# keeffEoghan/tendrils

Hardware: AMD Instinct MI355X
Metric: particle-steps/sec (16M particles per GPU) (higher is better)
Workload: dtype f32

## Files before the change

include/tendrils_hip.h:

```cpp
#ifndef TENDRILS_HIP_H
#define TENDRILS_HIP_H

#include <stddef.h>
#include <stdint.h>

#ifdef __cplusplus
extern "C" {
#endif

#define TH_ABI_VERSION 14

typedef int32_t th_status;
enum {
    TH_OK = 0,
    TH_ERR_INVALID = 1,
    TH_ERR_HIP = 2,
    TH_ERR_NO_DEVICE = 3,
    TH_ERR_UNSUPPORTED = 4
};

#define TH_INERT (-1000000.0f)

typedef struct th_context th_context;

// ... 171 lines not shown
} th_render_uniforms;
th_status th_view_draw(th_context *ctx, const th_render_uniforms *u, uint64_t *fragments);
th_status th_draw(th_context *ctx, const th_deposit_uniforms *u, const th_render_uniforms *r, uint64_t *fragments);
th_status th_view_fill(th_context *ctx, const float rgba[4]);
th_status th_view_clear(th_context *ctx);
th_status th_view_download(th_context *ctx, uint8_t *rgba8);
th_status th_view_buffers(th_context *ctx, int32_t count);
th_status th_view_bind(th_context *ctx, int32_t index);
th_status th_view_copy(th_context *ctx, int32_t index);
th_status th_view_step_buffers(th_context *ctx);
th_status th_colormap_upload(th_context *ctx, const float *rgba, int32_t w, int32_t h);
th_status th_export_view_lines(th_context *ctx, const th_render_uniforms *u, float *lines, uint64_t capacity, uint64_t *count);
th_status th_draw_sharded(th_context *ctx, const th_deposit_uniforms *u, const th_render_uniforms *r, uint64_t *fragments);
th_status th_view_emit(th_context *ctx, const th_render_uniforms *u, uint64_t *count, void **keys_dev, void **colors_dev);
th_status th_view_merge(th_context *ctx, const void *keys_dev, const void *colors_dev, uint64_t count);
th_status th_view_device_ptr(th_context *ctx, void **dptr);
th_status th_draw_emit(th_context *ctx, const th_deposit_uniforms *u, const th_render_uniforms *r, uint64_t *count, void **keys_dev, void **colors_dev);
th_status th_draw_merge(th_context *ctx, const void *keys_dev, const void *colors_dev, uint64_t count);

typedef struct th_slot_order_info {
    int32_t sorted_buffers;
    int32_t steps_since_sort;
    uint64_t window_misses;
    uint64_t sorts;
} th_slot_order_info;
th_status th_slot_order(th_context *ctx, th_slot_order_info *out);

enum { TH_DRAW_AUTO = -1, TH_DRAW_STREAM = 0, TH_DRAW_BINS = 1 };
th_status th_draw_pipeline(th_context *ctx, int32_t which);
typedef struct th_draw_info {
    int32_t pipeline;
    int32_t reserved;
    uint64_t fragments, crowded_fragments;
    uint64_t sent_bytes, received_bytes;
} th_draw_info;
th_status th_draw_query(th_context *ctx, th_draw_info *out);

typedef struct th_flow_line_uniforms {
    float speed, rad, crestShape, speedLimit;
    float viewSize[2];
} th_flow_line_uniforms;

th_status th_flow_line_attributes(const float *points, const double *times, int32_t n, int32_t closed, int32_t capacity,
                                  int32_t *nverts, float *position, float *normal, float *miter, float *previous,
                                  float *time, float *dt);
th_status th_flow_lines(th_context *ctx, const th_flow_line_uniforms *u, const float *points, const double *times,
                        const int32_t *offsets, const int32_t *closed, int32_t nlines);

enum { TH_OPT_BUCKET = 0, TH_OPT_RESORT_STEPS = 1, TH_OPT_REBUCKET_STEPS = 2, TH_OPT_FUSE = 3, TH_OPT_GRAPH = 4,
       TH_OPT_FORCE_GENERIC = 5, TH_OPT_DRAW_REUSE = 6, TH_OPT_BINS_POOL = 7,
#ifdef TH_TESTING
       TH_OPT_INJECT_FAILURE = 8,
#endif
       TH_OPT_BINS_PAGES = 9, TH_OPT_ASYNC_SORT = 10, TH_OPT_SKIP_UNSEEN = 11, TH_OPT_SPAWN_CHUNK_ROWS = 12 };
th_status th_option_set(th_context *ctx, int32_t option, int64_t value);
th_status th_option_get(th_context *ctx, int32_t option, int64_t *value);

#ifdef __cplusplus
}
#endif
#endif
```

tendrils_amd/csrc/th_api.hip:

```cpp
#include "th_ctx.hpp"

using namespace thi;

namespace {

thread_local std::string g_error;

void build_gradient_table(float4 *lut)
{
    for (int a = th::kLutMin; a <= th::kLutMax; ++a) {
        float p = th::permute_ref((float)a);
        float gx, gy, gz;
        th::gradient_ref(p, gx, gy, gz);
        lut[a - th::kLutMin] = make_float4(gx, gy, gz, 0.0f);
    }
}

void options_from_environment(th_options &o)
{
    auto number = [](const char *name, long long otherwise) { const char *e = getenv(name); return e && *e ? atoll(e) : otherwise; };
    o.bucket = (int)number("TH_BUCKET", -1);
    o.resort_steps = (int)number("TH_RESORT_STEPS", 64); if (o.resort_steps <= 0) o.resort_steps = 64;
    o.rebucket_steps = (int)number("TH_REBUCKET_STEPS", 256); if (o.rebucket_steps <= 0) o.rebucket_steps = 256;
    o.fuse = number("TH_FUSE", 1) != 0;
    o.graph = number("TH_GRAPH", 1) != 0;
    o.force_generic = getenv("TH_FORCE_GENERIC") != nullptr && number("TH_FORCE_GENERIC", 1) != 0;
    const char *d = getenv("TH_DRAW");
    o.draw = !d ? -1 : (!strcmp(d, "bins") ? 1 : (!strcmp(d, "stream") ? 0 : -1));
    o.draw_reuse = number("TH_DRAW_REUSE", 1) != 0;
    o.async_sort = number("TH_ASYNC_SORT", 1) != 0;
    o.skip_unseen = number("TH_SKIP_UNSEEN", 1) != 0;
    o.spawn_chunk_rows = (int)number("TH_SPAWN_CHUNK_ROWS", 0); if (o.spawn_chunk_rows < 0) o.spawn_chunk_rows = 0;
    o.bins_pool = (uint32_t)number("TH_BINS_POOL", 0);
    o.bins_pages = (int)number("TH_BINS_PAGES", 0); if (o.bins_pages > (int)th::kBinPagesLimit || o.bins_pages < -(int)th::kBinPagesLimit) o.bins_pages = 0;
}

}

namespace thi {

std::string &last_error() { return g_error; }

th_status fail(th_status code, const char *fmt, ...)
{
    char buf[512];
    va_list ap;
    va_start(ap, fmt);
    vsnprintf(buf, sizeof buf, fmt, ap);
    va_end(ap);
    g_error = buf;
    return code;
}

th_status use(th_context *c, bool keeps_lines)
{
    if (!c) return fail(TH_ERR_INVALID, "null context");
    TH_HIP(hipSetDevice(c->cfg.device));
    if (!keeps_lines) { c->drawn.valid = false; c->fused_stats.valid = false; }
    return TH_OK;
}

th_status alloc_state(th_context *c, float4 **out)
{
    TH_HIP(hipMalloc((void **)out, c->state_bytes()));
    TH_HIP(hipMemsetAsync(*out, 0, c->state_bytes(), c->stream));
    return TH_OK;
}

th_status resolve_target(th_context *c, int32_t target, bool rotate_ok, float4 **out)
{
    if (target == TH_TARGET_RING) {
        if (!rotate_ok) return fail(TH_ERR_INVALID, "TH_TARGET_RING not valid here");
        float4 *last = c->ring.back();
        c->ring.pop_back();
        c->ring.insert(c->ring.begin(), last);
        *out = c->ring[0];
        state_written(c, *out);
// ... 462 lines not shown
th_status th_timer_stop(th_context *c, float *elapsed_ms)
{
    if (th_status s = use(c, true)) return s;
    TH_REQUIRE(elapsed_ms, "null output");
    TH_HIP(hipEventRecord(c->ev1, c->stream));
    TH_HIP(hipEventSynchronize(c->ev1));
    TH_HIP(hipEventElapsedTime(elapsed_ms, c->ev0, c->ev1));
    return TH_OK;
}

th_status th_kernel_timing(th_context *c, int32_t enable)
{
    if (th_status s = use(c, true)) return s;
    c->kernel_timing = enable != 0;
    if (!enable) c->kt_used = 0;
    return TH_OK;
}

th_status th_kernel_timing_read(th_context *c, float *mean_ms, int32_t *launches)
{
    if (th_status s = use(c, true)) return s;
    TH_REQUIRE(mean_ms && launches, "null output");
    TH_HIP(hipStreamSynchronize(c->stream));
    double sum = 0.0;
    for (size_t k = 0; k + 1 < c->kt_used; k += 2) {
        float ms = 0.0f;
        TH_HIP(hipEventElapsedTime(&ms, c->kt_events[k], c->kt_events[k + 1]));
        sum += ms;
    }
    *launches = (int32_t)(c->kt_used / 2);
    *mean_ms = *launches ? (float)(sum / *launches) : 0.0f;
    c->kt_used = 0;
    return TH_OK;
}

th_status th_shapes(th_context *c, th_shapes_info *out)
{
    TH_REQUIRE(c && out, "null argument");
    out->state_w = c->cfg.width; out->state_h = c->cfg.height;
    out->flow_w = c->fw; out->flow_h = c->fh;
    out->frames_w = c->frw; out->frames_h = c->frh;
    return TH_OK;
}

th_status th_option_set(th_context *c, int32_t option, int64_t value)
{
    if (th_status s = use(c)) return s;
    th_options &o = c->opt;
    switch (option) {
    case TH_OPT_BUCKET: TH_REQUIRE(value >= -1 && value <= 1, "TH_OPT_BUCKET takes -1, 0 or 1"); o.bucket = (int)value; break;
    case TH_OPT_RESORT_STEPS: TH_REQUIRE(value > 0 && value < (1 << 30), "TH_OPT_RESORT_STEPS must be positive"); o.resort_steps = (int)value; break;
    case TH_OPT_REBUCKET_STEPS: TH_REQUIRE(value > 0 && value < (1 << 30), "TH_OPT_REBUCKET_STEPS must be positive"); o.rebucket_steps = (int)value; break;
    case TH_OPT_FUSE: o.fuse = value != 0; break;
    case TH_OPT_GRAPH: o.graph = value != 0; break;
    case TH_OPT_FORCE_GENERIC: o.force_generic = value != 0; break;
    case TH_OPT_DRAW_REUSE: o.draw_reuse = value != 0; break;
    case TH_OPT_SKIP_UNSEEN: o.skip_unseen = value != 0; break;
    case TH_OPT_ASYNC_SORT: o.async_sort = value != 0; if (!o.async_sort) { if (th_status s = asort_drop(c)) return s; } break;
    case TH_OPT_BINS_POOL: TH_REQUIRE(value >= 0 && value < (1ll << 32), "TH_OPT_BINS_POOL out of range"); o.bins_pool = (uint32_t)value; break;
#ifdef TH_TESTING
    case TH_OPT_INJECT_FAILURE: TH_REQUIRE(value >= 0 && value <= 5, "TH_OPT_INJECT_FAILURE takes 0..5"); o.inject_failure = (int)value; break;
#endif
    case TH_OPT_SPAWN_CHUNK_ROWS: TH_REQUIRE(value >= 0 && value < (1 << 30), "TH_OPT_SPAWN_CHUNK_ROWS takes 0 (by the scratch budget) or a number of rows"); o.spawn_chunk_rows = (int)value; break;
    case TH_OPT_BINS_PAGES:
        TH_REQUIRE(value >= -(int64_t)th::kBinPagesLimit && value <= (int64_t)th::kBinPagesLimit && value != 1 && value != -1, "TH_OPT_BINS_PAGES takes 0, or 2..%u (negative: never widened)", th::kBinPagesLimit);
        o.bins_pages = (int)value;
        if (c->chunk_table) {
            TH_HIP(hipStreamSynchronize(c->stream));
            (void)hipFree(c->chunk_table); c->chunk_table = nullptr; (void)hipFree(c->bin_mem); c->bin_mem = nullptr; c->bin_capacity = 0; c->bin_max_pages = 0;
        }
        break;
    default: return fail(TH_ERR_INVALID, "unknown option %d", option);
    }
    clear_graphs(c);
    return TH_OK;
}

th_status th_option_get(th_context *c, int32_t option, int64_t *value)
{
    TH_REQUIRE(c && value, "null argument");
    const th_options &o = c->opt;
    switch (option) {
    case TH_OPT_BUCKET: *value = o.bucket; break;
    case TH_OPT_RESORT_STEPS: *value = o.resort_steps; break;
    case TH_OPT_REBUCKET_STEPS: *value = o.rebucket_steps; break;
    case TH_OPT_FUSE: *value = o.fuse; break;
    case TH_OPT_GRAPH: *value = o.graph; break;
    case TH_OPT_FORCE_GENERIC: *value = o.force_generic; break;
    case TH_OPT_DRAW_REUSE: *value = o.draw_reuse; break;
    case TH_OPT_ASYNC_SORT: *value = o.async_sort; break;
    case TH_OPT_SKIP_UNSEEN: *value = o.skip_unseen; break;
    case TH_OPT_BINS_POOL: *value = o.bins_pool; break;
#ifdef TH_TESTING
    case TH_OPT_INJECT_FAILURE: *value = o.inject_failure; break;
#endif
    case TH_OPT_BINS_PAGES: *value = o.bins_pages; break;
    case TH_OPT_SPAWN_CHUNK_ROWS: *value = o.spawn_chunk_rows; break;
    default: return fail(TH_ERR_INVALID, "unknown option %d", option);
    }
    return TH_OK;
}

}
```

tendrils_amd/csrc/th_ctx.hpp:

```cpp
#pragma once
#include <hip/hip_runtime.h>

#include <algorithm>
#include <cmath>
#include <cstdarg>
#include <cstdio>
#include <cstdlib>
#include <cstring>
#include <limits>
#include <new>
#include <string>
#include <vector>

#include "th_kernels.hpp"
#include "th_math.hpp"

namespace thi {
struct FlowLineScratch;
th_status fail(th_status code, const char *fmt, ...);
std::string &last_error();
}

#define TH_HIP(expr)                                                                            \
    do {                                                                                        \
        hipError_t e_ = (expr);                                                                 \
        if (e_ != hipSuccess)                                                                   \
            return thi::fail(TH_ERR_HIP, "%s failed: %s (%s:%d)", #expr, hipGetErrorString(e_), __FILE__, __LINE__); \
    } while (0)

#define TH_REQUIRE(cond, ...)                            \
    do {                                                 \
        if (!(cond)) return thi::fail(TH_ERR_INVALID, __VA_ARGS__); \
    } while (0)

struct th_options {
    int bucket = -1;
    int resort_steps = 64;
    int rebucket_steps = 256;
    bool fuse = true;
    bool graph = true;
    bool force_generic = false;
    int draw = -1;
    bool draw_reuse = true;
    uint32_t bins_pool = 0;
    int bins_pages = 0;
    int inject_failure = 0;
    bool skip_unseen = true;
    int spawn_chunk_rows = 0;
    bool async_sort = true;
};

struct GraphEntry {
    int32_t n = 0;
    th::LogicVariant variant{};
    bool generic = false;
    std::vector<float4 *> ring;
    th::LogicParams key{};
    hipGraphExec_t exec = nullptr;
    float *times_dev = nullptr, *times_host = nullptr;
    hipEvent_t copied = nullptr;
};

struct th_context {
    th_config cfg{};
    th_options opt{};
    hipStream_t stream = nullptr;
    std::vector<float4 *> ring;
    bool packed = false;
    float4 *tmp[3] = {nullptr, nullptr, nullptr};
    float4 *flow = nullptr;
    float2 *flow_dec = nullptr;
    float *flow3 = nullptr;
    int32_t fw = 0, fh = 0;
    float4 *targets = nullptr;
    bool targets_checked = true, targets_nonfinite = false;
    float4 *lut = nullptr, *lut_block = nullptr;
    uchar4 *frames[2] = {nullptr, nullptr};
    int32_t frw = 0, frh = 0;
    unsigned int *d_flag = nullptr;
    th::StatsPartial *partials = nullptr;
    th::StatsPartial *fused_parts = nullptr;
    uint32_t fused_parts_cap = 0;
    struct { bool valid = false; const float4 *buf = nullptr; float limit = 0.0f; uint32_t nparts = 0; } fused_stats;
    th_counters *d_counters = nullptr;
    float4 *x_halo = nullptr;
    unsigned long long *x_counts = nullptr;
    unsigned long long *x_keys = nullptr;
    float4 *x_colors = nullptr;
    size_t x_capacity = 0;
    float4 *gathered = nullptr;
    const void *gathered_of = nullptr;
    void *sp_taps = nullptr;
// ... 208 lines not shown
```

tendrils_amd/csrc/th_kernels.hip:

```cpp
#include "th_kernels.hpp"
#include "th_math.hpp"
#include "th_logic.hpp"

#include <type_traits>
#include <cstdlib>

namespace th {


static int grid_for(size_t n, int blocks_per_cu)
{
    size_t blocks = (n + 255) / 256;
    size_t cap = (size_t)256 * blocks_per_cu;
    return (int)(blocks < cap ? (blocks ? blocks : 1) : cap);
}



__global__ __launch_bounds__(256) void pack_state_kernel(uint2 *dst, const float4 *src, uint32_t n)
{
    for (uint32_t i = blockIdx.x * 256u + threadIdx.x; i < n; i += gridDim.x * 256u) dst[i] = pack_state(src[i]);
}

__global__ __launch_bounds__(256) void unpack_state_kernel(float4 *dst, const uint2 *src, uint32_t n)
// ... 102 lines not shown
    if (b) lift([&](auto... c) { f(std::true_type{}, c...); }, rest...);
    else lift([&](auto... c) { f(std::false_type{}, c...); }, rest...);
}

void launch_logic(const LogicParams &p, const LogicVariant &v, hipStream_t s)
{
    const bool packed = v.format == StateFormat::packed;
    const int grid = packed ? grid_for(p.count, p.perm ? 20 : 8) : grid_for(p.count, 20);
    lift([&](auto fast, auto noise, auto target, auto pow2, auto decoded, auto perm) {
        constexpr bool ptab = noise && perm;
        hipLaunchKernelGGL((packed ? logic_packed_kernel<fast, noise, target, pow2, decoded, ptab>
                                   : logic_kernel<fast, noise, target, pow2, decoded, ptab>), dim3(grid), dim3(256), 0, s, p);
    }, v.mode == TH_MODE_FAST, v.noise, v.target, v.pow2, v.decoded, p.perm != nullptr);
}

void launch_logic_generic(const LogicParams &p, hipStream_t s)
{
    hipLaunchKernelGGL(logic_generic_kernel, dim3(grid_for(p.count, 8)), dim3(256), 0, s, p);
}

TH_D void stats_take(StatsPartial *slot, const float4 &v, float limit, bool first)
{
    const float cap = limit * (1.0f - 9.5367431640625e-07f);
    const bool is_live = v.x != kInert || v.y != kInert;
    const bool is_nan = (v.x != v.x) || (v.y != v.y) || (v.z != v.z) || (v.w != v.w);
    const float sp = __builtin_sqrtf(v.z * v.z + v.w * v.w);
    const bool fin = is_live && !is_nan && sp <= 3.4028234e38f;
    StatsPartial t;
    t.live = __builtin_popcountll(__ballot(is_live)); t.nan = __builtin_popcountll(__ballot(is_nan));
    t.capped = __builtin_popcountll(__ballot(fin && sp >= cap));
    double sum = fin ? (double)sp : 0.0;
    float mx = fin ? sp : 0.0f;
#pragma unroll
    for (int o = 32; o > 0; o >>= 1) {
        sum += __shfl_xor(sum, o);
        const float om = __shfl_xor(mx, o); mx = om > mx ? om : mx;
    }
    if (__lane_id() == (uint32_t)__builtin_ctzll(__ballot(true))) {
        t.sum_speed = sum; t.max_speed = (double)mx;
        if (!first) {
            const StatsPartial o = *slot;
            t.live += o.live; t.nan += o.nan; t.capped += o.capped; t.sum_speed += o.sum_speed;
            t.max_speed = o.max_speed > t.max_speed ? o.max_speed : t.max_speed;
        }
        *slot = t;
    }
}

TH_D void stats_none(StatsPartial *slot, bool first)
{
    if (__ballot(!first) == 0ull && __lane_id() == 0u) *slot = StatsPartial{0ull, 0ull, 0ull, 0.0, 0.0};
}

#define TH_LOGIC_FUSED_LOOP(Fmt)                                                                                              \
    __shared__ float4 smem[NOISE ? kHashVec + kLutSize : 1];                                                                  \
    const float4 *lut = smem + (NOISE ? kHashVec : 0);                                                                        \
    const HashTables tabs{reinterpret_cast<const uint32_t *>(smem), reinterpret_cast<const uint32_t *>(smem) + kPermA};       \
    if constexpr (NOISE) {                                                                                                    \
        fill_hash_tables(smem, p.lut);                                                                                        \
        __syncthreads();                                                                                                      \
    }                                                                                                                         \
    uint32_t idx, stride, end;                                                                                                \
    if constexpr (!BUCKETED) {                                                                                                \
        idx = blockIdx.x * 256u + threadIdx.x;                                                                                \
        stride = gridDim.x * 256u;                                                                                            \
        end = p.count;                                                                                                        \
    } else {                                                                                                                  \
        const uint32_t group = blockIdx.x & 7u, rank = blockIdx.x >> 3, per = (p.count + 7u) >> 3;                            \
        const uint32_t lo = group * per;                                                                                      \
        idx = lo + rank * 256u + threadIdx.x;                                                                                 \
        stride = (gridDim.x >> 3) * 256u;                                                                                     \
        end = lo + per < p.count ? lo + per : p.count;                                                                        \
    }                                                                                                                         \
    typename Fmt::Word nxt = Fmt::empty();                                                                                    \
    uint32_t npid = idx;                                                                                                      \
    [[maybe_unused]] bool first = true;                                                                                       \
    if (idx < end) {                                                                                                          \
        nxt = Fmt::load(p.in, idx);                                                                                           \
        if constexpr (BUCKETED) npid = __builtin_nontemporal_load(&p.perm[idx]);                                              \
    }                                                                                                                         \
    for (; idx < end; idx += stride) {                                                                                        \
        typename Fmt::Word w = nxt, wprev = w;                                                                                \
        const uint32_t pid = BUCKETED ? npid : idx;                                                                           \
        if (idx + stride < end) {                                                                                             \
            nxt = Fmt::load(p.in, idx + stride);                                                                              \
            if constexpr (BUCKETED) npid = __builtin_nontemporal_load(&p.perm[idx + stride]);                                 \
        }                                                                                                                     \
        float4 st = Fmt::decode(w);                                                                                           \
        for (uint32_t k = 0; k < p.nsteps; ++k) {                                                                             \
            if constexpr (!Fmt::packed) wprev = Fmt::encode(st);                                                              \
            else if (k + 1u == p.nsteps && k) wprev = Fmt::encode(st);                                                        \
            st = Fmt::quantize(integrate<FAST, NOISE, TARGET, POW2, false, true, !NOISE>(p, lut, st, pid, p.times[k], &tabs)); \
        }                                                                                                                     \
        if (!Fmt::packed || p.nsteps) w = Fmt::encode(st);                                                                    \
        Fmt::store(p.out_prev, idx, wprev);                                                                                   \
        Fmt::store(p.out, idx, w);                                                                                            \
        if constexpr (STATS) { stats_take(&p.stats_part[blockIdx.x * 4u + (threadIdx.x >> 6)], st, p.u.speedLimit, first); first = false; } \
    }                                                                                                                         \
    if constexpr (STATS) stats_none(&p.stats_part[blockIdx.x * 4u + (threadIdx.x >> 6)], first);

template <bool FAST, bool NOISE, bool TARGET, bool POW2, bool BUCKETED, bool STATS>
__global__ __launch_bounds__(256) void logic_fused_kernel(const LogicParams p) { TH_LOGIC_FUSED_LOOP(F32Texel) }

template <bool FAST, bool NOISE, bool TARGET, bool POW2, bool BUCKETED, bool STATS>
__global__ __launch_bounds__(256, 5) void logic_fused_packed_kernel(const LogicParams p) { TH_LOGIC_FUSED_LOOP(PackedTexel) }

static int fused_grid(uint32_t count, bool bucketed)
{
    const uint32_t blocks = (count + 255u) / 256u;
    const uint32_t grid = bucketed ? 8u * ((((count + 7u) >> 3) + 255u) / 256u) : blocks;
    return (int)(grid ? grid : 1u);
}

void launch_logic_fused(const LogicParams &p, const LogicVariant &v, hipStream_t s)
{
    const bool packed = v.format == StateFormat::packed, bucketed = p.perm != nullptr;
    const int grid = fused_grid(p.count, bucketed);
    lift([&](auto fast, auto noise, auto target, auto pow2, auto bk, auto stats) {
        hipLaunchKernelGGL((packed ? logic_fused_packed_kernel<fast, noise, target, pow2, bk, stats>
                                   : logic_fused_kernel<fast, noise, target, pow2, bk, stats>), dim3(grid), dim3(256), 0, s, p);
    }, v.mode == TH_MODE_FAST, v.noise, v.target, v.pow2, bucketed, p.stats_part != nullptr);
}

TH_D uint32_t tile_key(const TileGeom &g, float px, float py, uint32_t pid)
{
    const uint32_t row = g.row0 + (g.pow2w ? pid >> g.log2w : pid / g.width);
    const uint32_t idle = ((g.row_draws[row >> 5] >> (row & 31u)) & 1u) ^ 1u;
    const bool taps = __builtin_fabsf(px) < __builtin_inff() && __builtin_fabsf(py) < __builtin_inff() &&
                      (px != kInert || py != kInert);
    if (!taps) return 2u * g.ntiles + idle;
    const int tx = (int)__builtin_amdgcn_fmed3f((px * g.view_x + 1.0f) * g.half_fw, 0.0f, g.fwm1);
    const int ty = (int)__builtin_amdgcn_fmed3f((py * g.view_y + 1.0f) * g.half_fh, 0.0f, g.fhm1);
    return 2u * ((uint32_t)(ty >> kTileShift) * g.tiles_x + (uint32_t)(tx >> kTileShift)) + idle;
}

struct WaveRuns { bool head; uint32_t rank, length, head_lane; };
TH_D WaveRuns wave_runs(uint32_t key, bool valid)
{
    const uint32_t lane = __lane_id();
    const uint32_t prev = __shfl_up(key, 1);
    const unsigned long long vmask = __ballot(valid);
    const bool head = valid && (lane == 0 || key != prev);
    const unsigned long long heads = __ballot(head);
    WaveRuns r;
    r.head = head;
    const unsigned long long below = heads & ((2ull << lane) - 1ull);
    r.head_lane = below ? 63u - (uint32_t)__builtin_clzll(below) : 0u;
    r.rank = lane - r.head_lane;
    const unsigned long long above = lane < 63u ? (heads >> (lane + 1u)) : 0ull;
    const uint32_t next = above ? lane + 1u + (uint32_t)__builtin_ctzll(above) : (uint32_t)__builtin_popcountll(vmask);
    r.length = next - lane;
    return r;
}

constexpr uint32_t kBinEmpty = 0xffffffffu;
struct ChunkBins { uint32_t key[kBinSlots], count[kBinSlots], base[kBinSlots]; };

TH_D void bins_clear(ChunkBins &t)
{
    if (threadIdx.x < kBinSlots) { t.key[threadIdx.x] = kBinEmpty; t.count[threadIdx.x] = 0u; t.base[threadIdx.x] = 0u; }
}
TH_D int bins_slot(ChunkBins &t, uint32_t key, bool insert)
{
    uint32_t h = (key * 2654435761u) >> (32 - kBinSlotsLog2);
    for (uint32_t n = 0; n < kBinSlots; ++n, h = (h + 1u) & (kBinSlots - 1u)) {
        const uint32_t k = *(volatile uint32_t *)&t.key[h];
        if (k == key) return (int)h;
        if (k == kBinEmpty) {
            if (!insert) return -1;
            const uint32_t old = atomicCAS(&t.key[h], kBinEmpty, key);
            if (old == kBinEmpty || old == key) return (int)h;
        }
    }
// ... 873 lines not shown
            c.sum_speed += sh[w].sum_speed;
            c.max_speed = sh[w].max_speed > c.max_speed ? sh[w].max_speed : c.max_speed;
        }
        *out = c;
    }
}

__global__ __launch_bounds__(256) void stats_fold_parts_kernel(const StatsPartial *part, uint32_t nparts, StatsPartial *out)
{
    __shared__ StatsPartial sh[4];
    const uint32_t k = blockIdx.x * 256u + threadIdx.x;
    StatsPartial a = k < nparts ? part[k] : StatsPartial{0, 0, 0, 0.0, 0.0};
#pragma unroll
    for (int o = 32; o > 0; o >>= 1) {
        a.live += __shfl_xor(a.live, o); a.nan += __shfl_xor(a.nan, o); a.capped += __shfl_xor(a.capped, o);
        a.sum_speed += __shfl_xor(a.sum_speed, o);
        const double om = __shfl_xor(a.max_speed, o); a.max_speed = om > a.max_speed ? om : a.max_speed;
    }
    if ((threadIdx.x & 63) == 0) sh[threadIdx.x >> 6] = a;
    __syncthreads();
    if (threadIdx.x == 0) {
        StatsPartial t = sh[0];
        for (int w = 1; w < 4; ++w) {
            t.live += sh[w].live; t.nan += sh[w].nan; t.capped += sh[w].capped;
            t.sum_speed += sh[w].sum_speed; t.max_speed = sh[w].max_speed > t.max_speed ? sh[w].max_speed : t.max_speed;
        }
        out[blockIdx.x] = t;
    }
}

uint32_t fused_stats_parts(uint32_t count, bool sorted) { return 4u * (uint32_t)fused_grid(count, sorted); }

void launch_stats_fold(const StatsPartial *parts, uint32_t nparts, StatsPartial *scratch, size_t n, const unsigned long long *respawned,
                       th_counters *out, hipStream_t s)
{
    while (nparts > 4096u) {
        const uint32_t blocks = (nparts + 255u) / 256u;
        hipLaunchKernelGGL(stats_fold_parts_kernel, dim3(blocks), dim3(256), 0, s, parts, nparts, scratch);
        parts = scratch; scratch += blocks; nparts = blocks;
    }
    hipLaunchKernelGGL(stats_fold_kernel, dim3(1), dim3(256), 0, s, parts, (int)nparts, n, respawned, out);
}

void launch_stats(const float4 *state, size_t n, float speed_limit, StatsPartial *partials,
                  const unsigned long long *respawned, th_counters *out, hipStream_t s)
{
    int grid = grid_for(n, 4);
    if (grid > kStatsBlocks) grid = kStatsBlocks;
    hipLaunchKernelGGL(stats_kernel, dim3(grid), dim3(256), 0, s, state, n, speed_limit, partials);
    hipLaunchKernelGGL(stats_fold_kernel, dim3(1), dim3(256), 0, s, partials, grid, n, respawned, out);
}

}
```

tendrils_amd/csrc/th_kernels.hpp:

```cpp
#pragma once
#include <string>

#include <hip/hip_runtime.h>
#include <stdint.h>

#include "../../include/tendrils_hip.h"

namespace th {

constexpr uint32_t kMaxFusedSteps = 32;

constexpr uint32_t kTileChunk = 4096;
constexpr uint32_t kMaxTileBins = 8192;
constexpr uint32_t kSortReplicas = 64;
constexpr uint32_t kBinSlotsLog2 = 6, kBinSlots = 1u << kBinSlotsLog2;

struct TileGeom {
    float view_x, view_y, half_fw, half_fh, fwm1, fhm1;
    uint32_t tiles_x, ntiles;
    uint32_t width, log2w, pow2w, row0;
    const uint32_t *row_draws;
};

struct TileChunk { uint32_t start, count, tile, pad; };
struct ChunkRecord { uint32_t key[kBinSlots], count[kBinSlots]; };

struct LogicParams {
    const float4 *in;
    float4 *out;
    const float4 *flow;
    const float2 *flow_dec;
    const float *flow3;
    const float4 *targets;
    const float4 *lut;
    uint32_t count;
    uint32_t width;
    uint32_t log2w;
    uint32_t row0;
    float wf, hf;
    float inv_w, inv_h, inv_wh;
    int32_t fw, fh;
    float fwf, fhf, fwm1, fhm1, half_fw, half_fh;
    th_logic_uniforms u;
    float s2_cap;
    float pos_bound;
    const uint32_t *perm;
    TileGeom geom;
    const TileChunk *chunks;
    const uint32_t *nchunks;
    uint32_t *cursor;
    uint32_t *perm_out;
    float4 *in_moved;
    uint32_t *hist;
    ChunkRecord *records;
    uint32_t use_records;
    const float *time_dev;
    uint8_t *seen;
    float seen_xlo, seen_xhi, seen_ylo, seen_yhi;
    float4 *out_prev;
    uint32_t nsteps;
    struct StatsPartial *stats_part;
    float times[kMaxFusedSteps];
};

struct TileSortParams {
    const float4 *state;
    const uint32_t *perm_in;
    uint32_t count;
    TileGeom g;
    uint32_t *hist;
    uint32_t *cursor;
    uint32_t *totals, *starts;
    TileChunk *chunks;
    uint32_t *nchunks;
    float4 *state_out;
    uint32_t *perm_out;
    ChunkRecord *block_records;
    uint32_t packed;
};

struct OpticalFlowParams {
    const uchar4 *view, *last;
    float4 *flow;
    int32_t fr_w, fr_h;
    int32_t out_w, out_h;
    float grad_x, grad_y;
    th_optical_flow_uniforms u;
};

struct SpawnBallParams {
    float4 *out;
    uint32_t count, width, row0;
    th_spawn_ball_uniforms u;
};

struct SpawnSampleParams {
    const float4 *particles;
    float4 *out;
    const float4 *data;
    uint32_t count, width, row0;
    float wf, hf;
    int32_t dw, dh;
    th_spawn_sample_uniforms u;
    unsigned long long *accepted;
};

struct SpawnShardParams {
    const float4 *particles;
    float4 *out;
    const float4 *data;
    uint32_t first, count;
    uint32_t width, row0, rows, global_rows;
    float wf, hf;
    uint32_t world, base, extra;
// ... 234 lines not shown
```

tendrils_amd/csrc/th_logic.hpp:

```cpp
#pragma once
#include "th_kernels.hpp"
#include "th_math.hpp"

namespace th {

typedef float v4f __attribute__((ext_vector_type(4)));
typedef unsigned v2u __attribute__((ext_vector_type(2)));
typedef float v2f __attribute__((ext_vector_type(2)));

TH_D uint32_t mad_u24_s(uint32_t a, uint32_t b, uint32_t c)
{
    uint32_t r;
    asm("v_mad_u32_u24 %0, %1, %2, %3" : "=v"(r) : "v"(a), "s"(b), "v"(c));
    return r;
}

TH_D float4 load_stream(const float4 *p)
{
    v4f v = __builtin_nontemporal_load(reinterpret_cast<const v4f *>(p));
    return make_float4(v.x, v.y, v.z, v.w);
}
TH_D void store_stream(float4 *p, float4 a)
{
    v4f v = {a.x, a.y, a.z, a.w};
// ... 51 lines not shown
    float fcx = (float)x + 0.5f, fcy = (float)y_global + 0.5f;
    float uvx = fcx / p.wf, uvy = fcy / p.hf;
    float posx = st.x, posy = st.y, velx = st.z, vely = st.w;
    if (!(posx != kInert || posy != kInert)) return st;

    float i = (fcx + (fcy * p.wf)) / (p.wf * p.hf);
    float nscale = vary(u.noiseScale, i, u.varyNoiseScale);
    float nx = posx * nscale, ny = posy * nscale;
    float ntime = time * vary(u.noiseSpeed, i, u.varyNoiseSpeed);
    float wx = snoise_ref(nx, ny, uvx + ntime);
    float wy = snoise_ref(nx, ny, uvy + ntime + 1234.5678f);

    float sx = posx * u.viewSize[0], sy = posy * u.viewSize[1];
    float fu = 0.0f + (1.0f * (sx + 1.0f)) / 2.0f;
    float fv = 0.0f + (1.0f * (sy + 1.0f)) / 2.0f;
    int tx = (int)__builtin_amdgcn_fmed3f(th_floor(fu * p.fwf), 0.0f, p.fwm1);
    int ty = (int)__builtin_amdgcn_fmed3f(th_floor(fv * p.fhf), 0.0f, p.fhm1);
    float4 ft = p.flow[(size_t)ty * p.fw + tx];
    float k = __builtin_fmaxf(0.0f, 1.0f - ((time - ft.z) * u.flowDecay));
    float ffx = (0.0f + ft.x * k * 1.0f) / 1.0f, ffy = (0.0f + ft.y * k * 1.0f) / 1.0f;

    float vfw = vary(u.forceWeight, i, u.varyForce);
    float vflw = vary(u.flowWeight, i, u.varyFlow);
    float vnw = vary(u.noiseWeight, i, u.varyNoise);
    float nvx = (velx * u.damping * u.dt) + (vfw * ((ffx * u.dt * vflw) + (wx * u.dt * vnw)));
    float nvy = (vely * u.damping * u.dt) + (vfw * ((ffy * u.dt * vflw) + (wy * u.dt * vnw)));

    float4 tg = p.targets[local_index];
    float vtg = vary(u.target, i, u.varyTarget);
    nvx += (tg.x - posx) * vtg;
    nvy += (tg.y - posy) * vtg;

    float speed = __builtin_sqrtf(nvx * nvx + nvy * nvy);
    float r = __builtin_fminf(speed, u.speedLimit) / speed;
    nvx *= r; nvy *= r;
    return make_float4(posx + nvx, posy + nvy, nvx, nvy);
}

struct NoiseCorners {
    float ax, ay, az, bx, by, bz, cx, cy, cz, dx, dy, dz;
    int j0, j1, j2, j3;
};

constexpr uint32_t kBiasBitsA = 0x4A000000u, kBiasBitsB = 0x49000000u;
constexpr int kPermA = 292, kPermB = 584;
constexpr int kHashVec = (kPermA + kPermB) / 4;
struct HashTables {
    const uint32_t *permA, *permB;
};

TH_D void fill_hash_tables(float4 *smem, const float4 *lut_global)
{
    const float4 *block = lut_global - kHashVec;
    for (int k = threadIdx.x; k < kHashVec + kLutSize; k += 256) smem[k] = block[k];
}


template <bool FAST>
TH_D NoiseCorners snoise_corners_tab(float vx, float vy, float vz, float sxy, const HashTables &T)
{
    NoiseCorners n;
    float s = mad<FAST>(vz, kC3, sxy);
    float ix = th_floor(vx + s), iy = th_floor(vy + s), iz = th_floor(vz + s);
    float t = mad<FAST>(iz, kC6, mad<FAST>(iy, kC6, ix * kC6));
    float ax = (vx - ix) + t, ay = (vy - iy) + t, az = (vz - iz) + t;

    const float ax1 = ax - 1.0f, ay1 = ay - 1.0f, az1 = az - 1.0f;
    float bx, by, bz, cx, cy, cz;
    uint32_t e1x, e2x, e1y, e2y;
    unsigned long long mz1, mz2;
    {
        unsigned long long l1, l2, l3, m;
        asm("v_cmp_lt_f32 %[l1], %[ax], %[ay]\n\t"
            "v_cmp_lt_f32 %[l2], %[ay], %[az]\n\t"
            "v_cmp_lt_f32 %[l3], %[az], %[ax]\n\t"
            "s_andn2_b64 %[m], %[l3], %[l1]\n\t"     "v_cndmask_b32 %[bx], %[ax], %[ax1], %[m]\n\t"   "v_cndmask_b32 %[e1x], 0, 16, %[m]\n\t"
            "s_andn2_b64 %[m], %[l1], %[l2]\n\t"     "v_cndmask_b32 %[by], %[ay], %[ay1], %[m]\n\t"   "v_cndmask_b32 %[e1y], 0, 4, %[m]\n\t"
            "s_andn2_b64 %[mz1], %[l2], %[l3]\n\t"   "v_cndmask_b32 %[bz], %[az], %[az1], %[mz1]\n\t"
            "s_orn2_b64 %[m], %[l3], %[l1]\n\t"      "v_cndmask_b32 %[cx], %[ax], %[ax1], %[m]\n\t"   "v_cndmask_b32 %[e2x], 0, 16, %[m]\n\t"
            "s_orn2_b64 %[m], %[l1], %[l2]\n\t"      "v_cndmask_b32 %[cy], %[ay], %[ay1], %[m]\n\t"   "v_cndmask_b32 %[e2y], 0, 4, %[m]\n\t"
            "s_orn2_b64 %[mz2], %[l2], %[l3]\n\t"    "v_cndmask_b32 %[cz], %[az], %[az1], %[mz2]"
            : [l1] "=&s"(l1), [l2] "=&s"(l2), [l3] "=&s"(l3), [m] "=&s"(m), [mz1] "=&s"(mz1), [mz2] "=&s"(mz2),
              [bx] "=&v"(bx), [by] "=&v"(by), [bz] "=&v"(bz), [cx] "=&v"(cx), [cy] "=&v"(cy), [cz] "=&v"(cz),
              [e1x] "=&v"(e1x), [e2x] "=&v"(e2x), [e1y] "=&v"(e1y), [e2y] "=&v"(e2y)
            : [ax] "v"(ax), [ay] "v"(ay), [az] "v"(az), [ax1] "v"(ax1), [ay1] "v"(ay1), [az1] "v"(az1)
            : "scc");
    }
    n.ax = ax; n.ay = ay; n.az = az;
    n.bx = bx + kC6; n.by = by + kC6; n.bz = bz + kC6;
    n.cx = cx + kC3; n.cy = cy + kC3; n.cz = cz + kC3;
    n.dx = ax - 0.5f; n.dy = ay - 0.5f; n.dz = az - 0.5f;

    uint32_t zb, yb, xb;
    asm("v_add_f32 %0, 0x4a000000, %1" : "=v"(zb) : "v"(mod289_int(iz)));
    asm("v_add_f32 %0, 0x4a000000, %1" : "=v"(yb) : "v"(mod289_int(iy)));
    asm("v_add_f32 %0, 0x49000000, %1" : "=v"(xb) : "v"(mod289_int(ix)));
    zb &= 0xffcu;
    const uint32_t *pa = reinterpret_cast<const uint32_t *>(reinterpret_cast<const char *>(T.permA) + zb);
    const uint32_t a0 = pa[0] + yb, a1 = pa[1] + yb;
    uint32_t sel1, sel2;
    asm("v_cndmask_b32 %0, %2, %3, %4\n\tv_cndmask_b32 %1, %2, %3, %5"
        : "=&v"(sel1), "=&v"(sel2) : "v"(a0), "v"(a1), "s"(mz1), "s"(mz2));
    auto stage_y = [&](uint32_t off) { return *reinterpret_cast<const uint32_t *>(reinterpret_cast<const char *>(T.permB) + off); };
    const uint32_t q0 = stage_y(a0), q1 = stage_y(sel1 + e1y), q2 = stage_y(sel2 + e2y), q3 = stage_y(a1 + 4u);
    n.j0 = (int)(q0 + xb); n.j1 = (int)(q1 + (xb + e1x)); n.j2 = (int)(q2 + (xb + e2x)); n.j3 = (int)(q3 + xb + 16u);
    return n;
}
// ... 202 lines not shown
```

tendrils_amd/csrc/th_step.hip:

```cpp
#include "th_ctx.hpp"

using namespace thi;

namespace {

float s2_cap_for(float limit)
{
    if (!(limit > 0.0f)) return -1.0f;
    if (std::isinf(limit)) return std::numeric_limits<float>::max();
    double sq = (double)limit * (double)limit;
    if (sq >= (double)std::numeric_limits<float>::max()) return std::numeric_limits<float>::max();
    float c = (float)sq;
    while (sqrtf(c) > limit) c = nextafterf(c, 0.0f);
    for (;;) {
        float n = nextafterf(c, std::numeric_limits<float>::infinity());
        if (std::isinf(n) || sqrtf(n) > limit) break;
        c = n;
    }
    return c;
}

bool finite_uniforms(const th_logic_uniforms &u)
{
    const float *f = reinterpret_cast<const float *>(&u);
// ... 274 lines not shown
    th_logic_uniforms v = *u;
    v.dt = (float)dt_ms;
    std::vector<float> times((size_t)n);
    double t = time0, tmax = 0.0;
    for (int32_t k = 0; k < n; ++k) {
        t += dt_ms;
        times[(size_t)k] = (float)t;
        if (std::fabs(t) > std::fabs(tmax)) tmax = t;
    }
    v.time = (float)tmax;
    StepPlan plan;
    if (th_status s = plan_step(c, v, TH_TARGET_RING, plan)) return s;

    if (c->opt.fuse && n >= 2 && c->ring.size() == 2 && !plan.generic) {
        if (plan.may_sort) {
            const th::TileGeom g = tile_geom(c, plan.p.u);
            int o = order_of(c, c->ring[0]);
            const bool stale = o >= 0 && (!same_geom(c->orders[(size_t)o].geom, g) || c->orders[(size_t)o].fw != c->fw ||
                                          c->orders[(size_t)o].fh != c->fh);
            if (o < 0 || stale || c->steps_since_sort >= c->opt.rebucket_steps) {
                float4 *cur = c->ring[0], *other = c->ring[1];
                set_order(c, other, -1);
                int fresh = -1;
                th::TileSortParams b;
                if (th_status s = begin_sort(c, g, cur, o >= 0 ? c->orders[(size_t)o].perm : nullptr, &fresh, &b)) return s;
                b.state_out = other;
                th::launch_tile_scatter(b, c->stream);
                TH_HIP(hipGetLastError());
                set_order(c, other, fresh);
                set_order(c, cur, -1);
                state_written(c, other); state_moved(c, cur, other);
                c->ring[0] = other; c->ring[1] = cur;
            }
        } else if (th_status s = ensure_identity(c)) return s;
        const bool pack3 = th::fused_taps_flow3(plan.v);
        if (pack3) {
            if (!c->flow3) TH_HIP(hipMalloc((void **)&c->flow3, (size_t)c->fw * c->fh * 3 * sizeof(float)));
            th::launch_flow_pack3(c->flow, c->flow3, (size_t)c->fw * c->fh, c->stream);
        }
        {
            int32_t done = 0;
            while (done < n) {
                const int32_t m = std::min<int32_t>(n - done, (int32_t)th::kMaxFusedSteps);
                th::LogicParams p = plan.p;
                p.flow3 = pack3 ? c->flow3 : nullptr;
                float4 *cur = c->ring[0], *other = c->ring[1];
                const int order = order_of(c, cur);
                state_written(c, cur); state_written(c, other);
                p.in = cur;
                p.out = (m & 1) ? other : cur;
                p.out_prev = (m & 1) ? cur : other;
                p.perm = order >= 0 ? c->orders[(size_t)order].perm : nullptr;
                p.nsteps = (uint32_t)m;
                for (int32_t k = 0; k < m; ++k) p.times[k] = times[(size_t)(done + k)];
                const bool takes_stats = done + m == n;
                if (takes_stats) {
                    const uint32_t parts = th::fused_stats_parts(p.count, p.perm != nullptr), need = parts + (parts + 255u) / 256u + 16u;
                    if (c->fused_parts_cap < need) {
                        TH_HIP(hipStreamSynchronize(c->stream));
                        (void)hipFree(c->fused_parts); c->fused_parts = nullptr; c->fused_parts_cap = 0;
                        TH_HIP(hipMalloc((void **)&c->fused_parts, (size_t)need * sizeof(th::StatsPartial)));
                        c->fused_parts_cap = need;
                    }
                    p.stats_part = c->fused_parts;
                    c->fused_stats.nparts = parts; c->fused_stats.limit = p.u.speedLimit;
                }
                hipEvent_t k0 = nullptr, k1 = nullptr;
                if (c->kernel_timing) {
                    if (th_status s = timing_events(c, &k0, &k1)) return s;
                    TH_HIP(hipEventRecord(k0, c->stream));
                }
                th::launch_logic_fused(p, plan.v, c->stream);
                if (k1) TH_HIP(hipEventRecord(k1, c->stream));
                TH_HIP(hipGetLastError());
                set_order(c, other, order);
                c->counted.buf = nullptr;
                if (m & 1) { c->ring[0] = other; c->ring[1] = cur; }
                c->steps_since_sort += m; c->total_steps += m;
                done += m;
                if (takes_stats) { c->fused_stats.valid = true; c->fused_stats.buf = c->ring[0]; }
            }
            return TH_OK;
        }
    }

    if (th_status s = ensure_identity(c)) return s;
    if (!c->opt.graph || n < 2 || (c->packed && plan.generic)) {
        for (int32_t k = 0; k < n; ++k) {
            if (k) { v.time = times[(size_t)k]; if (th_status s = plan_step(c, v, TH_TARGET_RING, plan)) return s; }
            if (th_status s = enqueue_step(c, plan, TH_TARGET_RING, times[(size_t)k], nullptr, true)) return s;
        }
        return TH_OK;
    }

    th::LogicParams key = plan.p;
    key.u.time = 0.0f;
    GraphEntry *hit = nullptr;
    for (GraphEntry &g : c->graphs)
        if (g.n == n && g.variant == plan.v && g.generic == plan.generic && g.ring == c->ring && same_key(g.key, key)) { hit = &g; break; }
    if (!hit) {
        if (c->graphs.size() >= 8) { destroy_graph(c->graphs.front()); c->graphs.erase(c->graphs.begin()); }
        GraphEntry g;
        g.n = n; g.variant = plan.v; g.generic = plan.generic; g.ring = c->ring; g.key = key;
        TH_HIP(hipMalloc((void **)&g.times_dev, (size_t)n * sizeof(float)));
        TH_HIP(hipHostMalloc((void **)&g.times_host, (size_t)n * sizeof(float)));
        TH_HIP(hipEventCreate(&g.copied));
// ... 41 lines not shown
```

tendrils_amd/particles.py:

```python
import ctypes as C

import numpy as np

from . import _capi
from ._capi import call


def defaults():
    return dict(shape=[64, 64], geomShape=None,
                logic=None, logicVert=None, logicFrag=None,
                render=None, renderVert=None, renderFrag=None)


class Program:

    def __init__(self, kind, **fixed):
        self.kind = kind
        self.fixed = fixed
        self.uniforms = {}

    def bind(self):
        return self


# ... 94 lines not shown
        call("th_upload_state", self._ctx, int(buffer), t.ctypes.data_as(_capi._fp), 0, 0,
             self.shape[0], self.shape[1])

    def read(self, buffer=0):
        index = buffer.index if isinstance(buffer, StateBuffer) else int(buffer)
        out = np.empty((self.shape[1], self.shape[0], 4), np.float32)
        call("th_download_state", self._ctx, index, out.ctypes.data_as(_capi._fp), 0, 0,
             self.shape[0], self.shape[1])
        return out

    def _target_index(self, buffer):
        if buffer is None:
            return _capi.TH_TARGET_RING
        if isinstance(buffer, StateBuffer):
            return buffer.index
        return buffer.target_index()

    def step(self, update=None, buffer=None):
        target = self._target_index(buffer)
        uniforms = Particles.applyUpdate(
            dict(self.logic.uniforms, dataRes=self.shape, geomRes=self.geomShape), update)
        self.logic.uniforms = uniforms
        run_pass(self, self.logic, uniforms, target)
        if buffer is None:
            self.buffers.insert(0, self.buffers.pop())

    def step_n(self, update, time0, dt_ms, n):
        uniforms = Particles.applyUpdate(
            dict(self.logic.uniforms, dataRes=self.shape, geomRes=self.geomShape), update)
        self.logic.uniforms = uniforms
        if self.logic.kind != LOGIC:
            raise ValueError("step_n runs the logic program only")
        s = logic_uniforms(uniforms)
        call("th_step_n", self._ctx, C.byref(s), C.c_double(time0), C.c_double(dt_ms), int(n))
        for _ in range(int(n) % max(len(self.buffers), 1)):
            self.buffers.insert(0, self.buffers.pop())

    def draw(self, update=None, mode=None):
        return None

    def updateLogic(self, logicFrag):
        self.logic = logicFrag if isinstance(logicFrag, Program) else Program(LOGIC)

    def updateRender(self, *a):
        pass

    def sync(self):
        call("th_sync", self._ctx)

    def draw_pipeline(self, which):
        call("th_draw_pipeline", self._ctx, {"auto": -1, "stream": 0, "bins": 1}[which])

    OPTIONS = dict(bucket=0, resort_steps=1, rebucket_steps=2, fuse=3, graph=4, force_generic=5, draw_reuse=6, bins_pool=7,
                   inject_failure=8, bins_pages=9, async_sort=10, skip_unseen=11, spawn_chunk_rows=12)

    def option(self, name, value=None):
        if value is not None:
            call("th_option_set", self._ctx, self.OPTIONS[name], int(value))
        out = C.c_int64(0)
        call("th_option_get", self._ctx, self.OPTIONS[name], C.byref(out))
        return out.value

    def fetches_taps(self, source):
        if self.sharded_spawn != "auto":
            return bool(self.sharded_spawn)
        if source < 0 or self._global_height in (0, self.shape[1]):
            return False
        q = _capi.CommInfo()
        call("th_comm_query", self._ctx, C.byref(q))
        return bool(q.active)

    def deposit_flow(self, view_size, time, speed_limit):
        u = _capi.DepositUniforms(time=float(time), speedLimit=float(speed_limit))
        u.viewSize[0], u.viewSize[1] = float(view_size[0]), float(view_size[1])
        n = C.c_uint64(0)
        call("th_flow_deposit", self._ctx, C.byref(u), C.byref(n))
        return int(n.value)

    def export_lines(self, view_size, time, speed_limit):
        u = _capi.DepositUniforms(time=float(time), speedLimit=float(speed_limit))
        u.viewSize[0], u.viewSize[1] = float(view_size[0]), float(view_size[1])
        n = C.c_uint64(0)
        call("th_export_lines", self._ctx, C.byref(u), None, 0, C.byref(n))
        out = np.empty((int(n.value), 12), np.float32)
        if n.value:
            call("th_export_lines", self._ctx, C.byref(u), out.ctypes.data_as(_capi._fp), n.value, C.byref(n))
        return out

    def stats(self, speed_limit):
        c = _capi.Counters()
        call("th_stats", self._ctx, C.c_float(speed_limit), C.byref(c))
        return {k: getattr(c, k) for k, _ in _capi.Counters._fields_}

    @staticmethod
    def generateLUT(shape):
        w, h = max(shape[0], 2), max(shape[1], 2)
        inv_x, inv_y = 1 / (w - 1), 1 / (h - 1)
        data = np.zeros(shape[0] * shape[1] * 2, np.float32)
        k = 0
        for i in range(w):
            for j in range(h):
                if k + 1 < data.size:
                    data[k] = i * inv_x
                    data[k + 1] = j * inv_y
                k += 2
        return data

# ... 58 lines not shown
```

Baseline: 205.0 billion.

## Stagger fused-kernel wave starts and issue state loads before hash-table fill

Adds an opt-in option that makes each resident workgroup's waves sleep in proportion to their wave slot, spreading out start-up contention. In the stats variant, the first state and permutation loads are now issued before the shared-memory hash-table fill, so their latency overlaps the fill. The table fill loads every element into registers first and then stores them all to shared memory. A scheduling barrier is placed before the stats accumulation, and compile-time-gated timestamp instrumentation is added. The stagger is off by default, and the load reordering adds register pressure.

```diff
diff --git a/include/tendrils_hip.h b/include/tendrils_hip.h
--- a/include/tendrils_hip.h
+++ b/include/tendrils_hip.h
@@ -247,7 +247,7 @@
 #ifdef TH_TESTING
        TH_OPT_INJECT_FAILURE = 8,
 #endif
-       TH_OPT_BINS_PAGES = 9, TH_OPT_ASYNC_SORT = 10, TH_OPT_SKIP_UNSEEN = 11, TH_OPT_SPAWN_CHUNK_ROWS = 12 };
+       TH_OPT_BINS_PAGES = 9, TH_OPT_ASYNC_SORT = 10, TH_OPT_SKIP_UNSEEN = 11, TH_OPT_SPAWN_CHUNK_ROWS = 12, TH_OPT_FUSED_STAGGER = 13 };
 th_status th_option_set(th_context *ctx, int32_t option, int64_t value);
 th_status th_option_get(th_context *ctx, int32_t option, int64_t *value);
 
diff --git a/tendrils_amd/csrc/th_api.hip b/tendrils_amd/csrc/th_api.hip
--- a/tendrils_amd/csrc/th_api.hip
+++ b/tendrils_amd/csrc/th_api.hip
@@ -23,6 +23,7 @@
     o.resort_steps = (int)number("TH_RESORT_STEPS", 64); if (o.resort_steps <= 0) o.resort_steps = 64;
     o.rebucket_steps = (int)number("TH_REBUCKET_STEPS", 256); if (o.rebucket_steps <= 0) o.rebucket_steps = 256;
     o.fuse = number("TH_FUSE", 1) != 0;
+    o.fused_stagger = (int)number("TH_FUSED_STAGGER", 0); if (o.fused_stagger < 0 || o.fused_stagger > 1024) o.fused_stagger = 0;
     o.graph = number("TH_GRAPH", 1) != 0;
     o.force_generic = getenv("TH_FORCE_GENERIC") != nullptr && number("TH_FORCE_GENERIC", 1) != 0;
     const char *d = getenv("TH_DRAW");
@@ -591,6 +592,7 @@
     case TH_OPT_RESORT_STEPS: TH_REQUIRE(value > 0 && value < (1 << 30), "TH_OPT_RESORT_STEPS must be positive"); o.resort_steps = (int)value; break;
     case TH_OPT_REBUCKET_STEPS: TH_REQUIRE(value > 0 && value < (1 << 30), "TH_OPT_REBUCKET_STEPS must be positive"); o.rebucket_steps = (int)value; break;
     case TH_OPT_FUSE: o.fuse = value != 0; break;
+    case TH_OPT_FUSED_STAGGER: TH_REQUIRE(value >= 0 && value <= 1024, "TH_OPT_FUSED_STAGGER takes 0 (off) or 1..1024 units of 64 clocks"); o.fused_stagger = (int)value; break;
     case TH_OPT_GRAPH: o.graph = value != 0; break;
     case TH_OPT_FORCE_GENERIC: o.force_generic = value != 0; break;
     case TH_OPT_DRAW_REUSE: o.draw_reuse = value != 0; break;
@@ -624,6 +626,7 @@
     case TH_OPT_RESORT_STEPS: *value = o.resort_steps; break;
     case TH_OPT_REBUCKET_STEPS: *value = o.rebucket_steps; break;
     case TH_OPT_FUSE: *value = o.fuse; break;
+    case TH_OPT_FUSED_STAGGER: *value = o.fused_stagger; break;
     case TH_OPT_GRAPH: *value = o.graph; break;
     case TH_OPT_FORCE_GENERIC: *value = o.force_generic; break;
     case TH_OPT_DRAW_REUSE: *value = o.draw_reuse; break;
diff --git a/tendrils_amd/csrc/th_ctx.hpp b/tendrils_amd/csrc/th_ctx.hpp
--- a/tendrils_amd/csrc/th_ctx.hpp
+++ b/tendrils_amd/csrc/th_ctx.hpp
@@ -38,6 +38,7 @@
     int resort_steps = 64;
     int rebucket_steps = 256;
     bool fuse = true;
+    int fused_stagger = 0;
     bool graph = true;
     bool force_generic = false;
     int draw = -1;
diff --git a/tendrils_amd/csrc/th_kernels.hip b/tendrils_amd/csrc/th_kernels.hip
--- a/tendrils_amd/csrc/th_kernels.hip
+++ b/tendrils_amd/csrc/th_kernels.hip
@@ -178,14 +178,43 @@
     if (__ballot(!first) == 0ull && __lane_id() == 0u) *slot = StatsPartial{0ull, 0ull, 0ull, 0.0, 0.0};
 }
 
+TH_D void fused_stagger(const LogicParams &p)
+{
+    if (p.stagger == 0u || blockIdx.x >= p.stagger_resident) return;
+    const uint32_t slot = __builtin_amdgcn_s_getreg((3 << 11) | (0 << 6) | 4) & 0xfu;
+    for (uint32_t n = slot * p.stagger; n; --n) __builtin_amdgcn_s_sleep(1);
+}
+
+#ifdef TH_FUSED_STAMPS
+constexpr uint32_t kFusedStampWords = 5;
+__device__ unsigned long long *g_fused_stamps;
+__device__ unsigned int g_fused_stamp_waves;
+#define TH_FUSED_STAMP(k) unsigned long long stamp_[4]; stamp_[0] = stamp_[1] = stamp_[2] = 0ull; stamp_[k] = __builtin_amdgcn_s_memrealtime()
+#define TH_FUSED_STAMP_AFTER(k, value) do { asm volatile("" :: "v"(value)); stamp_[k] = __builtin_amdgcn_s_memrealtime(); } while (0)
+#define TH_FUSED_STAMP_END() do {                                                                                             \
+        stamp_[3] = __builtin_amdgcn_s_memrealtime();                                                                         \
+        const uint32_t wave_ = blockIdx.x * 4u + (threadIdx.x >> 6);                                                          \
+        if (g_fused_stamps && wave_ < g_fused_stamp_waves && (threadIdx.x & 63u) == 0u) {                                     \
+            unsigned long long *o_ = g_fused_stamps + (size_t)wave_ * kFusedStampWords;                                       \
+            const unsigned long long hw_ = __builtin_amdgcn_s_getreg((31 << 11) | (0 << 6) | 4);                              \
+            const unsigned long long xcc_ = __builtin_amdgcn_s_getreg((3 << 11) | (0 << 6) | 20) & 0xfu;                      \
+            if (stamp_[1] == 0ull) stamp_[1] = stamp_[2] = stamp_[3];                                                         \
+            o_[0] = stamp_[0]; o_[1] = stamp_[1]; o_[2] = stamp_[2]; o_[3] = stamp_[3]; o_[4] = hw_ | (xcc_ << 32);          \
+        }                                                                                                                     \
+    } while (0)
+#else
+#define TH_FUSED_STAMP(k) do {} while (0)
+#define TH_FUSED_STAMP_AFTER(k, value) do {} while (0)
+#define TH_FUSED_STAMP_END() do {} while (0)
+#endif
+
 #define TH_LOGIC_FUSED_LOOP(Fmt)                                                                                              \
+    TH_FUSED_STAMP(0);                                                                                                        \
+    constexpr bool kLoadsFirst = STATS;                                                                                       \
+    fused_stagger(p);                                                                                                         \
     __shared__ float4 smem[NOISE ? kHashVec + kLutSize : 1];                                                                  \
     const float4 *lut = smem + (NOISE ? kHashVec : 0);                                                                        \
     const HashTables tabs{reinterpret_cast<const uint32_t *>(smem), reinterpret_cast<const uint32_t *>(smem) + kPermA};       \
-    if constexpr (NOISE) {                                                                                                    \
-        fill_hash_tables(smem, p.lut);                                                                                        \
-        __syncthreads();                                                                                                      \
-    }                                                                                                                         \
     uint32_t idx, stride, end;                                                                                                \
     if constexpr (!BUCKETED) {                                                                                                \
         idx = blockIdx.x * 256u + threadIdx.x;                                                                                \
@@ -201,7 +230,15 @@
     typename Fmt::Word nxt = Fmt::empty();                                                                                    \
     uint32_t npid = idx;                                                                                                      \
     [[maybe_unused]] bool first = true;                                                                                       \
-    if (idx < end) {                                                                                                          \
+    if (kLoadsFirst && idx < end) {                                                                                           \
+        nxt = Fmt::load(p.in, idx);                                                                                           \
+        if constexpr (BUCKETED) npid = __builtin_nontemporal_load(&p.perm[idx]);                                              \
+    }                                                                                                                         \
+    if constexpr (NOISE) {                                                                                                    \
+        fill_hash_tables(smem, p.lut);                                                                                        \
+        __syncthreads();                                                                                                      \
+    }                                                                                                                         \
+    if (!kLoadsFirst && idx < end) {                                                                                          \
         nxt = Fmt::load(p.in, idx);                                                                                           \
         if constexpr (BUCKETED) npid = __builtin_nontemporal_load(&p.perm[idx]);                                              \
     }                                                                                                                         \
@@ -213,17 +250,21 @@
             if constexpr (BUCKETED) npid = __builtin_nontemporal_load(&p.perm[idx + stride]);                                 \
         }                                                                                                                     \
         float4 st = Fmt::decode(w);                                                                                           \
+        TH_FUSED_STAMP_AFTER(1, st.x);                                                                                        \
         for (uint32_t k = 0; k < p.nsteps; ++k) {                                                                             \
             if constexpr (!Fmt::packed) wprev = Fmt::encode(st);                                                              \
             else if (k + 1u == p.nsteps && k) wprev = Fmt::encode(st);                                                        \
-            st = Fmt::quantize(integrate<FAST, NOISE, TARGET, POW2, false, true, !NOISE>(p, lut, st, pid, p.times[k], &tabs)); \
+            st = Fmt::quantize(integrate<FAST, NOISE, TARGET, POW2, false, true, !NOISE>(p, lut, st, pid, p.times[k], &tabs));\
         }                                                                                                                     \
+        TH_FUSED_STAMP_AFTER(2, st.x);                                                                                        \
         if (!Fmt::packed || p.nsteps) w = Fmt::encode(st);                                                                    \
         Fmt::store(p.out_prev, idx, wprev);                                                                                   \
         Fmt::store(p.out, idx, w);                                                                                            \
-        if constexpr (STATS) { stats_take(&p.stats_part[blockIdx.x * 4u + (threadIdx.x >> 6)], st, p.u.speedLimit, first); first = false; } \
+        if constexpr (STATS) __builtin_amdgcn_sched_barrier(0);                                                               \
+        if constexpr (STATS) { stats_take(&p.stats_part[blockIdx.x * 4u + (threadIdx.x >> 6)], st, p.u.speedLimit, first); first = false; }\
     }                                                                                                                         \
-    if constexpr (STATS) stats_none(&p.stats_part[blockIdx.x * 4u + (threadIdx.x >> 6)], first);
+    if constexpr (STATS) stats_none(&p.stats_part[blockIdx.x * 4u + (threadIdx.x >> 6)], first);                              \
+    TH_FUSED_STAMP_END();
 
 template <bool FAST, bool NOISE, bool TARGET, bool POW2, bool BUCKETED, bool STATS>
 __global__ __launch_bounds__(256) void logic_fused_kernel(const LogicParams p) { TH_LOGIC_FUSED_LOOP(F32Texel) }
@@ -238,13 +279,28 @@
     return (int)(grid ? grid : 1u);
 }
 
+template <class K>
+static uint32_t resident_workgroups(K kernel)
+{
+    int dev = 0, cus = 0, per_cu = 0;
+    if (hipGetDevice(&dev) != hipSuccess || hipDeviceGetAttribute(&cus, hipDeviceAttributeMultiprocessorCount, dev) != hipSuccess ||
+        hipOccupancyMaxActiveBlocksPerMultiprocessor(&per_cu, kernel, 256, 0) != hipSuccess) { (void)hipGetLastError(); return 0u; }
+    return (uint32_t)(per_cu > 0 && cus > 0 ? per_cu * cus : 0);
+}
+
 void launch_logic_fused(const LogicParams &p, const LogicVariant &v, hipStream_t s)
 {
     const bool packed = v.format == StateFormat::packed, bucketed = p.perm != nullptr;
     const int grid = fused_grid(p.count, bucketed);
     lift([&](auto fast, auto noise, auto target, auto pow2, auto bk, auto stats) {
+        LogicParams q = p;
+        if (q.stagger) {
+            static const uint32_t resident[2] = {resident_workgroups(logic_fused_kernel<fast, noise, target, pow2, bk, stats>),
+                                                 resident_workgroups(logic_fused_packed_kernel<fast, noise, target, pow2, bk, stats>)};
+            q.stagger_resident = resident[packed];
+        }
         hipLaunchKernelGGL((packed ? logic_fused_packed_kernel<fast, noise, target, pow2, bk, stats>
-                                   : logic_fused_kernel<fast, noise, target, pow2, bk, stats>), dim3(grid), dim3(256), 0, s, p);
+                                   : logic_fused_kernel<fast, noise, target, pow2, bk, stats>), dim3(grid), dim3(256), 0, s, q);
     }, v.mode == TH_MODE_FAST, v.noise, v.target, v.pow2, bucketed, p.stats_part != nullptr);
 }
 
@@ -1224,3 +1280,30 @@
 }
 
 }
+
+#ifdef TH_FUSED_STAMPS
+static unsigned long long *g_fused_stamps_host_ptr = nullptr;
+static unsigned int g_fused_stamps_host_waves = 0;
+extern "C" int th_debug_fused_stamps_begin(unsigned int waves)
+{
+    unsigned long long *buf = nullptr;
+    const size_t bytes = (size_t)waves * th::kFusedStampWords * sizeof(unsigned long long);
+    if (g_fused_stamps_host_ptr || hipMalloc((void **)&buf, bytes) != hipSuccess) return 1;
+    if (hipMemset(buf, 0, bytes) != hipSuccess || hipMemcpyToSymbol(HIP_SYMBOL(th::g_fused_stamp_waves), &waves, sizeof waves) != hipSuccess ||
+        hipMemcpyToSymbol(HIP_SYMBOL(th::g_fused_stamps), &buf, sizeof buf) != hipSuccess) { (void)hipFree(buf); return 1; }
+    g_fused_stamps_host_ptr = buf; g_fused_stamps_host_waves = waves;
+    return 0;
+}
+extern "C" int th_debug_fused_stamps_read(unsigned long long *out, unsigned int waves)
+{
+    if (!g_fused_stamps_host_ptr || waves != g_fused_stamps_host_waves) return 1;
+    unsigned long long *none = nullptr;
+    const unsigned int zero = 0;
+    int bad = hipDeviceSynchronize() != hipSuccess;
+    bad |= hipMemcpy(out, g_fused_stamps_host_ptr, (size_t)waves * th::kFusedStampWords * sizeof(unsigned long long), hipMemcpyDeviceToHost) != hipSuccess;
+    bad |= hipMemcpyToSymbol(HIP_SYMBOL(th::g_fused_stamps), &none, sizeof none) != hipSuccess;
+    bad |= hipMemcpyToSymbol(HIP_SYMBOL(th::g_fused_stamp_waves), &zero, sizeof zero) != hipSuccess;
+    (void)hipFree(g_fused_stamps_host_ptr); g_fused_stamps_host_ptr = nullptr; g_fused_stamps_host_waves = 0;
+    return bad;
+}
+#endif
diff --git a/tendrils_amd/csrc/th_kernels.hpp b/tendrils_amd/csrc/th_kernels.hpp
--- a/tendrils_amd/csrc/th_kernels.hpp
+++ b/tendrils_amd/csrc/th_kernels.hpp
@@ -60,6 +60,8 @@
     float4 *out_prev;
     uint32_t nsteps;
     struct StatsPartial *stats_part;
+    uint32_t stagger;
+    uint32_t stagger_resident;
     float times[kMaxFusedSteps];
 };
 
diff --git a/tendrils_amd/csrc/th_logic.hpp b/tendrils_amd/csrc/th_logic.hpp
--- a/tendrils_amd/csrc/th_logic.hpp
+++ b/tendrils_amd/csrc/th_logic.hpp
@@ -127,7 +127,17 @@
 TH_D void fill_hash_tables(float4 *smem, const float4 *lut_global)
 {
     const float4 *block = lut_global - kHashVec;
-    for (int k = threadIdx.x; k < kHashVec + kLutSize; k += 256) smem[k] = block[k];
+    constexpr int kFill = kHashVec + kLutSize, kRounds = (kFill + 255) / 256;
+    float4 v[kRounds];
+    int at[kRounds];
+#pragma unroll
+    for (int r = 0; r < kRounds; ++r) {
+        const int k = (int)threadIdx.x + 256 * r;
+        at[r] = k < kFill - 1 ? k : kFill - 1;
+        v[r] = block[at[r]];
+    }
+#pragma unroll
+    for (int r = 0; r < kRounds; ++r) smem[at[r]] = v[r];
 }
 
 
diff --git a/tendrils_amd/csrc/th_step.hip b/tendrils_amd/csrc/th_step.hip
--- a/tendrils_amd/csrc/th_step.hip
+++ b/tendrils_amd/csrc/th_step.hip
@@ -350,6 +350,7 @@
                 p.out_prev = (m & 1) ? cur : other;
                 p.perm = order >= 0 ? c->orders[(size_t)order].perm : nullptr;
                 p.nsteps = (uint32_t)m;
+                p.stagger = (uint32_t)c->opt.fused_stagger;
                 for (int32_t k = 0; k < m; ++k) p.times[k] = times[(size_t)(done + k)];
                 const bool takes_stats = done + m == n;
                 if (takes_stats) {
diff --git a/tendrils_amd/particles.py b/tendrils_amd/particles.py
--- a/tendrils_amd/particles.py
+++ b/tendrils_amd/particles.py
@@ -170,7 +170,7 @@
         call("th_draw_pipeline", self._ctx, {"auto": -1, "stream": 0, "bins": 1}[which])
 
     OPTIONS = dict(bucket=0, resort_steps=1, rebucket_steps=2, fuse=3, graph=4, force_generic=5, draw_reuse=6, bins_pool=7,
-                   inject_failure=8, bins_pages=9, async_sort=10, skip_unseen=11, spawn_chunk_rows=12)
+                   inject_failure=8, bins_pages=9, async_sort=10, skip_unseen=11, spawn_chunk_rows=12, fused_stagger=13)
 
     def option(self, name, value=None):
         if value is not None:
```

After: 205.7 billion, median of 2. About the same (+0.4%).
